# microsoft/ctsTraffic

Measured on AMD Instinct MI355X. Metric: GiB/s verified, 64 KiB buffers device-resident; % MI355X HBM roofline, higher is better.
Workload: dtype u8

## Files before the change

ctstraffic_amd/csrc/cts_kernels.hip:

```cpp
#include <hip/hip_runtime.h>

#include <type_traits>

#include "cts_device_util.hpp"
#include "cts_grids.hpp"
#include "cts_internal.hpp"

namespace cts {

typedef uint32_t u32x4 __attribute__((ext_vector_type(4)));

__device__ __forceinline__ uint32_t pattern_byte_dev(uint32_t pos)
{
    pos &= 0xFFFFu;
    return (pos & 1u) ? (pos >> 9) : ((pos >> 1) & 0xFFu);
}

__device__ __forceinline__ u32x4 expected_chunk(uint32_t q, uint32_t sh)
{
    const uint32_t k = q >> 1;
    const uint32_t base = __umul24(k, 0x10001u) + 0x10000u;
    const uint32_t w0 = base & 0x7FFF7FFFu;
    const uint32_t w1 = (base + 0x20002u) & 0x7FFF7FFFu;
    const uint32_t w2 = (base + 0x40004u) & 0x7FFF7FFFu;
    const uint32_t w3 = (base + 0x60006u) & 0x7FFF7FFFu;
    const uint32_t w4 = (base + 0x80008u) & 0x7FFF7FFFu;
    return u32x4{__builtin_amdgcn_alignbyte(w1, w0, sh), __builtin_amdgcn_alignbyte(w2, w1, sh),
                 __builtin_amdgcn_alignbyte(w3, w2, sh), __builtin_amdgcn_alignbyte(w4, w3, sh)};
}

__device__ __forceinline__ uint32_t nonzero_bytes(uint32_t x)
{
    return (((x & 0x7F7F7F7Fu) + 0x7F7F7F7Fu) | x) & 0x80808080u;
}

__device__ __forceinline__ uint32_t low_bytes_mask(int nb)
{
    return (uint32_t)((1ull << (8 * nb)) - 1ull);
}

__device__ __forceinline__ u32x4 range_mask(uint32_t lo, uint32_t hi)
{
    u32x4 m;
#pragma unroll
    for (int w = 0; w < 4; ++w) {
        int a = (int)lo - 4 * w;
        int b = (int)hi - 4 * w;
        a = a < 0 ? 0 : (a > 4 ? 4 : a);
        b = b < 0 ? 0 : (b > 4 ? 4 : b);
        m[w] = (b > a) ? (low_bytes_mask(b) & ~low_bytes_mask(a)) : 0u;
    }
    return m;
}

template <bool NT>
__device__ __forceinline__ u32x4 load_chunk(const u32x4* p)
{
    if constexpr (NT) {
        return __builtin_nontemporal_load(p);
    } else {
        return *p;
    }
}

__device__ __forceinline__ uint32_t or4(u32x4 x) { return x[0] | x[1] | x[2] | x[3]; }

typedef const u32x4 __attribute__((address_space(1)))* gchunk_ptr;
template <bool NT>
__device__ __forceinline__ u32x4 load_chunk_g(const u32x4* p)
{
    const gchunk_ptr g = (gchunk_ptr)p;
    if constexpr (NT) {
        return __builtin_nontemporal_load(g);
    } else {
        return *g;
    }
}

struct Span {
    const u32x4* p;
    const uint8_t* sp;
    uint32_t len;
    uint32_t nchunks;
    uint32_t q0;
    uint32_t sh;
    uint32_t lo;
    uint32_t hi_last;
    uint32_t expected;
    uint32_t cb0;
};

__device__ __forceinline__ Span make_span(const uint8_t* __restrict__ arena, const cts_buf_desc& d)
{
    Span s;
    s.len = d.length - d.skip_head;
    s.sp = arena + d.byte_offset + d.skip_head;
    s.lo = (uint32_t)((uintptr_t)s.sp & 15u);
    s.nchunks = s.len == 0 ? 0u : (uint32_t)(((uint64_t)s.lo + s.len + 15u) >> 4);
    s.hi_last = s.len == 0 ? 0u : (uint32_t)((uint64_t)s.lo + s.len - 16ull * (s.nchunks - 1u));
    s.q0 = (d.expected_pattern_offset - s.lo) & 0xFFFFu;
    s.sh = s.q0 & 1u;
    s.p = reinterpret_cast<const u32x4*>(s.sp - s.lo);
    s.expected = d.expected_pattern_offset;
    const uint32_t a = (uint32_t)(((uintptr_t)s.p >> 4) & 7u);
    s.cb0 = 8u - a;
    return s;
}

__device__ __forceinline__ u32x4 chunk_xor(const Span& s, uint32_t c, u32x4 data)
{
    return data ^ expected_chunk((s.q0 + 16u * c) & 0xFFFFu, s.sh);
}

__device__ __forceinline__ u32x4 chunk_diff_masked(const Span& s, uint32_t c)
{
    u32x4 x = chunk_xor(s, c, s.p[c]);
    if (c == 0u || c == s.nchunks - 1u) x &= range_mask(c == 0u ? s.lo : 0u, c == s.nchunks - 1u ? s.hi_last : 16u);
    return x;
}

__device__ __forceinline__ __amdgpu_buffer_rsrc_t span_rsrc(const Span& s)
{
    return __builtin_amdgcn_make_buffer_rsrc(const_cast<u32x4*>(s.p), (short)0, (int)(s.nchunks * 16u), 0x00020000);
}

template <bool NT>
__device__ __forceinline__ u32x4 buf_load(__amdgpu_buffer_rsrc_t r, uint32_t voff, uint32_t soff)
{
    return __builtin_amdgcn_raw_buffer_load_b128(r, voff, soff, NT ? 2 : 0);
}

template <int TEAM, int U, bool EVEN = false>
__device__ __forceinline__ u32x4 expected_step(uint32_t B, int u, uint32_t sh)
{
    static_assert(32767 + 8 * TEAM * (U - 1) + 8 < 65536, "packed k must not carry");
    uint32_t bb = B;
    asm volatile("" : "+v"(bb));
    const uint32_t b = bb + (uint32_t)u * (uint32_t)(8 * TEAM) * 0x10001u;
    const uint32_t w0 = b & 0x7FFF7FFFu;
    const uint32_t w1 = (b + 0x20002u) & 0x7FFF7FFFu;
    const uint32_t w2 = (b + 0x40004u) & 0x7FFF7FFFu;
    const uint32_t w3 = (b + 0x60006u) & 0x7FFF7FFFu;
    if constexpr (EVEN) {
        return u32x4{w0, w1, w2, w3};
    } else {
        const uint32_t w4 = (b + 0x80008u) & 0x7FFF7FFFu;
        return u32x4{__builtin_amdgcn_alignbyte(w1, w0, sh), __builtin_amdgcn_alignbyte(w2, w1, sh),
                     __builtin_amdgcn_alignbyte(w3, w2, sh), __builtin_amdgcn_alignbyte(w4, w3, sh)};
    }
}

__device__ __forceinline__ uint32_t chunk_base(const Span& s, uint32_t c)
{
    const uint32_t k = ((s.q0 + 16u * c) & 0xFFFFu) >> 1;
    return __umul24(k, 0x10001u) + 0x10000u;
}

template <int TEAM, int U, bool NT, bool EVEN>
__device__ __forceinline__ uint32_t scan_rounds(const Span& s, __amdgpu_buffer_rsrc_t r, uint32_t lane, uint32_t cb,
                                                uint32_t c_end)
{
    uint32_t acc = 0;
    const uint32_t voff = lane * 16u;
    for (; cb + (uint32_t)(TEAM * U) <= c_end; cb += (uint32_t)(TEAM * U)) {
        u32x4 d[U];
#pragma unroll
        for (int u = 0; u < U; ++u) d[u] = buf_load<NT>(r, voff, (cb + (uint32_t)(u * TEAM)) * 16u);
        __builtin_amdgcn_sched_barrier(0);
        const uint32_t B = chunk_base(s, cb + lane);
#pragma unroll
        for (int u = 0; u < U; ++u) {
            acc |= or4(d[u] ^ expected_step<TEAM, U, EVEN>(B, u, s.sh));
            __builtin_amdgcn_sched_barrier(0);
        }
    }
    if (cb < c_end) {
        u32x4 d[U];
#pragma unroll
        for (int u = 0; u < U; ++u) d[u] = buf_load<NT>(r, (cb + (uint32_t)(u * TEAM) + lane) * 16u, 0u);
        __builtin_amdgcn_sched_barrier(0);
        const uint32_t B = chunk_base(s, cb + lane);
#pragma unroll
        for (int u = 0; u < U; ++u) {
            const uint32_t any = or4(d[u] ^ expected_step<TEAM, U, EVEN>(B, u, s.sh));
            acc |= (cb + (uint32_t)(u * TEAM) + lane < c_end) ? any : 0u;
            __builtin_amdgcn_sched_barrier(0);
        }
    }
    return acc;
}

template <int TEAM, int U, bool NT, bool EVEN>
__device__ __forceinline__ uint32_t scan_interior_impl(const Span& s, __amdgpu_buffer_rsrc_t r, uint32_t lane)
{
    if (s.nchunks < 3u) return 0;
    return scan_rounds<TEAM, U, NT, EVEN>(s, r, lane, s.cb0, s.nchunks - 1u);
}

template <int TEAM, int U, bool NT, bool SPLIT>
__device__ __forceinline__ uint32_t scan_interior(const Span& s, __amdgpu_buffer_rsrc_t r, uint32_t lane)
{
    if constexpr (SPLIT) {
        if (__builtin_amdgcn_readfirstlane(s.sh) == 0u) return scan_interior_impl<TEAM, U, NT, true>(s, r, lane);
    }
    return scan_interior_impl<TEAM, U, NT, false>(s, r, lane);
}

__device__ __forceinline__ bool span_whole_lines(const Span& s)
{
    return s.lo == 0u && s.hi_last == 16u && s.cb0 == 8u;
}

__device__ __forceinline__ uint32_t edge_chunk_of(const Span& s, uint32_t lane)
{
    return lane == 1u ? s.nchunks - 1u : ((lane >= 2u && lane <= 8u) ? lane - 1u : 0u);
}
__device__ __forceinline__ bool edge_chunk_used(const Span& s, uint32_t lane)
{
    if (s.nchunks == 0u) return false;
    if (lane == 0u) return true;
    if (lane == 1u) return s.nchunks > 1u;
    const uint32_t h = s.nchunks - 1u < s.cb0 ? s.nchunks - 1u : s.cb0;
    return lane >= 2u && lane <= 8u && lane - 1u < h;
}

template <int TEAM, int U, bool NT, bool SPLIT = false>
__device__ __forceinline__ uint32_t scan_buffer(const Span& s, uint32_t lane)
{
    const __amdgpu_buffer_rsrc_t r = span_rsrc(s);
    const uint32_t ce = edge_chunk_of(s, lane);
    const u32x4 edge = buf_load<NT>(r, edge_chunk_used(s, lane) ? ce * 16u : 0x7FFFFFF0u, 0u);
    uint32_t acc = scan_interior<TEAM, U, NT, SPLIT>(s, r, lane);
    const u32x4 x = chunk_xor(s, ce, edge) & range_mask(ce == 0u ? s.lo : 0u, ce == s.nchunks - 1u ? s.hi_last : 16u);
    acc |= edge_chunk_used(s, lane) ? or4(x) : 0u;
    return acc;
}

__device__ __forceinline__ void take_diff(const Span& s, uint32_t c, u32x4 x, uint32_t& first, uint32_t& count)
{
#pragma unroll
    for (int w = 0; w < 4; ++w) {
        const uint32_t nz = nonzero_bytes(x[w]);
        if (nz) {
            const uint32_t idx = 4u * (uint32_t)w + ((uint32_t)__builtin_ctz(nz) >> 3);
            const uint32_t pos = 16u * c + idx - s.lo;
            first = pos < first ? pos : first;
            count += (uint32_t)__builtin_popcount(nz);
        }
    }
}

template <int TEAM, int U, bool NT>
__device__ __forceinline__ void scan_exact_owned(const Span& s, uint32_t lane, uint32_t& first, uint32_t& count)
{
    if (s.nchunks == 0) return;
    const __amdgpu_buffer_rsrc_t r = span_rsrc(s);
    if (s.nchunks >= 3u) {
        const uint32_t c_end = s.nchunks - 1u;
        for (uint32_t cb = s.cb0; cb < c_end; cb += (uint32_t)(TEAM * U)) {
            u32x4 d[U];
#pragma unroll
            for (int u = 0; u < U; ++u) d[u] = buf_load<NT>(r, (cb + (uint32_t)(u * TEAM) + lane) * 16u, 0u);
#pragma unroll
            for (int u = 0; u < U; ++u) {
                const uint32_t c = cb + (uint32_t)(u * TEAM) + lane;
                if (c < c_end) take_diff(s, c, chunk_xor(s, c, d[u]), first, count);
            }
        }
    }
    if (edge_chunk_used(s, lane)) {
        const uint32_t c = edge_chunk_of(s, lane);
        const u32x4 x = chunk_xor(s, c, buf_load<NT>(r, c * 16u, 0u)) &
                        range_mask(c == 0u ? s.lo : 0u, c == s.nchunks - 1u ? s.hi_last : 16u);
        take_diff(s, c, x, first, count);
    }
}

template <int TEAM, int U, bool EVEN>
__device__ __forceinline__ void whole_exact_round(const Span& s, u32x4 (&d)[U], uint32_t cb, uint32_t lane,
                                                  uint32_t& first, uint32_t& count)
{
    const uint32_t B = chunk_base(s, cb + lane);
    uint32_t any = 0;
#pragma unroll
    for (int u = 0; u < U; ++u) {
        d[u] ^= expected_step<TEAM, U, EVEN>(B, u, s.sh);
        any |= or4(d[u]);
        __builtin_amdgcn_sched_barrier(0);
    }
    if (any != 0u) {
#pragma unroll
        for (int u = 0; u < U; ++u) take_diff(s, cb + (uint32_t)(u * TEAM) + lane, d[u], first, count);
    }
}

template <int TEAM, int U, bool NT, bool EVEN>
__device__ __forceinline__ void scan_whole_exact_impl(const Span& s, __amdgpu_buffer_rsrc_t r, uint32_t lane,
                                                      uint32_t& first, uint32_t& count)
{
    const uint32_t voff = lane * 16u;
    uint32_t cb = 0;
    const uint32_t c_end = s.nchunks;
    for (; cb + (uint32_t)(TEAM * U) <= c_end; cb += (uint32_t)(TEAM * U)) {
        u32x4 d[U];
#pragma unroll
        for (int u = 0; u < U; ++u) d[u] = buf_load<NT>(r, voff, (cb + (uint32_t)(u * TEAM)) * 16u);
        __builtin_amdgcn_sched_barrier(0);
        whole_exact_round<TEAM, U, EVEN>(s, d, cb, lane, first, count);
    }
    if (cb < c_end) {
        u32x4 d[U];
#pragma unroll
        for (int u = 0; u < U; ++u) d[u] = buf_load<NT>(r, (cb + (uint32_t)(u * TEAM) + lane) * 16u, 0u);
        __builtin_amdgcn_sched_barrier(0);
        const uint32_t B = chunk_base(s, cb + lane);
        uint32_t any = 0;
#pragma unroll
        for (int u = 0; u < U; ++u) {
            const bool in = cb + (uint32_t)(u * TEAM) + lane < c_end;
            d[u] = in ? (d[u] ^ expected_step<TEAM, U, EVEN>(B, u, s.sh)) : u32x4{0u, 0u, 0u, 0u};
            any |= or4(d[u]);
            __builtin_amdgcn_sched_barrier(0);
        }
        if (any != 0u) {
#pragma unroll
            for (int u = 0; u < U; ++u) take_diff(s, cb + (uint32_t)(u * TEAM) + lane, d[u], first, count);
        }
    }
}

template <int TEAM, int U, bool NT, bool SPLIT>
__device__ __forceinline__ void scan_whole_exact(const Span& s, uint32_t lane, uint32_t& first, uint32_t& count)
{
    const __amdgpu_buffer_rsrc_t r = span_rsrc(s);
    if constexpr (SPLIT) {
        if (__builtin_amdgcn_readfirstlane(s.sh) == 0u) {
            scan_whole_exact_impl<TEAM, U, NT, true>(s, r, lane, first, count);
            return;
        }
    }
    scan_whole_exact_impl<TEAM, U, NT, false>(s, r, lane, first, count);
}

constexpr uint32_t kGiantChunks = 1u << 27;

__device__ __forceinline__ bool span_giant(const Span& s)
{
    return __builtin_amdgcn_readfirstlane(s.nchunks >= kGiantChunks ? 1u : 0u) != 0u;
}

template <int TEAM, bool NT, uint32_t G = 2>
__device__ __forceinline__ void scan_giant_exact(const Span& s, uint32_t lane, uint32_t& first, uint32_t& count)
{
    for (uint32_t cb = 0; cb < s.nchunks; cb += G * TEAM) {
        u32x4 d[G];
#pragma unroll
        for (uint32_t g = 0; g < G; ++g) {
            const uint32_t c = cb + g * TEAM + lane;
            d[g] = load_chunk_g<NT>(s.p + (c < s.nchunks ? c : 0u));
        }
#pragma unroll
        for (uint32_t g = 0; g < G; ++g) {
            const uint32_t c = cb + g * TEAM + lane;
            if (c < s.nchunks) {
                u32x4 x = chunk_xor(s, c, d[g]);
                if (c == 0u || c == s.nchunks - 1u)
                    x &= range_mask(c == 0u ? s.lo : 0u, c == s.nchunks - 1u ? s.hi_last : 16u);
                take_diff(s, c, x, first, count);
            }
        }
    }
}

__device__ __forceinline__ uint32_t wave_min(uint32_t v)
{
#pragma unroll
    for (int off = 32; off > 0; off >>= 1) {
        const uint32_t o = (uint32_t)__shfl_xor((int)v, off, 64);
        v = o < v ? o : v;
    }
    return v;
}

__device__ __forceinline__ void write_bad(cts_verify_result* results, uint32_t i)
{
    if (results != nullptr) {
        cts_verify_result r;
        r.first_mismatch = 0;
        r.mismatch_bytes = 0;
        r.expected = 0;
        r.actual = 0;
        r.pass = 0;
        r.flags = CTS_RESULT_FLAG_BAD_DESC;
        results[i] = r;
    }
}

__device__ __forceinline__ void finish_buffer(const Span& s, const cts_buf_desc& d, uint32_t i, uint32_t first,
                                              uint32_t count, cts_verify_result* results, uint64_t* tc,
                                              uint32_t* conn_first_fail, uint32_t n_conns,
                                              cts_verify_result* rslot = nullptr, uint32_t base_index = 0u)
{
    const bool pass = (first == kNone);
    if (rslot != nullptr) {
        cts_verify_result r;
        r.first_mismatch = pass ? s.len : first;
        r.mismatch_bytes = pass ? 0u : count;
        r.expected = pass ? 0 : (uint8_t)pattern_byte_dev(s.expected + first);
        r.actual = pass ? 0 : s.sp[first];
        r.pass = pass ? 1 : 0;
        r.flags = 0;
        *rslot = r;
    } else if (results != nullptr) {
        cts_verify_result r;
        r.first_mismatch = pass ? s.len : first;
        r.mismatch_bytes = pass ? 0u : count;
        r.expected = pass ? 0 : (uint8_t)pattern_byte_dev(s.expected + first);
        r.actual = pass ? 0 : s.sp[first];
        r.pass = pass ? 1 : 0;
        r.flags = 0;
        results[i] = r;
    }
    tc[kBytesChecked] += s.len;
    tc[kBuffersChecked] += 1;
    if (pass) {
        tc[kBytesOk] += s.len;
    } else {
        tc[kBuffersFailed] += 1;
        tc[kMismatchedBytes] += count;
        if (conn_first_fail != nullptr && d.conn_index < n_conns &&
            atomicMin(&conn_first_fail[d.conn_index], base_index + i) == 0xFFFFFFFFu)
            tc[kConnectionsFailed] += 1;
    }
}

template <int TEAMS>
__device__ __forceinline__ void zero_counters(uint64_t (*ctr)[kCounterCount])
{
    if (threadIdx.x < (unsigned)(TEAMS * kCounterCount)) ctr[threadIdx.x / kCounterCount][threadIdx.x % kCounterCount] = 0;
    __syncthreads();
}

template <int TEAMS>
__device__ __forceinline__ void flush_counters(uint64_t* counters, uint64_t (*ctr)[kCounterCount])
{
    __syncthreads();
    if (counters == nullptr) return;
    if (threadIdx.x < (unsigned)kCounterCount) {
        uint64_t sum = 0;
#pragma unroll
        for (int t = 0; t < TEAMS; ++t) sum += ctr[t][threadIdx.x];
        if (sum)
            atomicAdd((unsigned long long*)&counters[(blockIdx.x % CTS_COUNTER_SHARDS) * kCounterSlots + threadIdx.x],
                      (unsigned long long)sum);
    }
}

__device__ __forceinline__ void block_reduce_mismatch_with(uint32_t& first, uint32_t& count, uint32_t* red)
{
    const uint32_t wave = threadIdx.x / 64;
    first = wave_min(first);
    count = wave_sum(count);
    if ((threadIdx.x & 63) == 0) {
        red[wave] = first;
        red[kBlock / 64 + wave] = count;
    }
    __syncthreads();
    if (threadIdx.x == 0) {
#pragma unroll
        for (int w = 1; w < kBlock / 64; ++w) {
            first = red[w] < first ? red[w] : first;
            count += red[kBlock / 64 + w];
        }
    }
    __syncthreads();
}

__device__ __forceinline__ void block_reduce_mismatch(uint32_t& first, uint32_t& count)
{
    __shared__ uint32_t red[2 * (kBlock / 64)];
    block_reduce_mismatch_with(first, count, red);
}

constexpr int kWgLoads = 2;

template <bool NT>
__device__ __forceinline__ void verify_wg_body(const uint8_t* __restrict__ arena, uint64_t arena_bytes,
                                               const cts_buf_desc* __restrict__ descs, uint32_t n,
                                               cts_verify_result* __restrict__ results, uint64_t* __restrict__ counters,
                                               uint32_t* __restrict__ conn_first_fail, uint32_t n_conns,
                                               uint32_t base_index)
{
    __shared__ uint64_t ctr[1][kCounterCount];
    const uint32_t lane = threadIdx.x;
    zero_counters<1>(ctr);
    const uint32_t step = gridDim.x;
    uint32_t i = blockIdx.x;
    cts_buf_desc dn;
    if (i < n) dn = descs[i];
    for (; i < n; i = (uint64_t)i + step < n ? i + step : n) {
        const cts_buf_desc d = dn;
        if ((uint64_t)i + step < n) dn = descs[i + step];
        if (desc_bad(d, arena_bytes)) {
            if (lane == 0) write_bad(results, i);
            continue;
        }
        const Span s = make_span(arena, d);
        uint32_t first = kNone, count = 0;
        bool dirty;
        if (span_giant(s)) {
            scan_giant_exact<kBlock, NT>(s, lane, first, count);
            dirty = __builtin_amdgcn_readfirstlane(__syncthreads_or(first != kNone)) != 0;
            if (dirty) block_reduce_mismatch(first, count);
        } else if (__builtin_amdgcn_readfirstlane(span_whole_lines(s) ? 1u : 0u)) {
            scan_whole_exact<kBlock, kWgLoads, NT, true>(s, lane, first, count);
            dirty = __builtin_amdgcn_readfirstlane(__syncthreads_or(first != kNone)) != 0;
            if (dirty) block_reduce_mismatch(first, count);
        } else {
            const uint32_t acc = scan_buffer<kBlock, kWgLoads, NT, true>(s, lane);
            dirty = __builtin_amdgcn_readfirstlane(__syncthreads_or(acc != 0u)) != 0;
            if (dirty) {
                if (acc != 0u) scan_exact_owned<kBlock, 2, NT>(s, lane, first, count);
                block_reduce_mismatch(first, count);
            }
        }
        if (lane == 0)
            finish_buffer(s, d, i, first, count, results, ctr[0], conn_first_fail, n_conns, nullptr, base_index);
    }
    flush_counters<1>(counters, ctr);
}

template <bool NT>
__global__ void __launch_bounds__(kBlock, 4)
    verify_wg_kernel(const uint8_t* __restrict__ arena, uint64_t arena_bytes, const cts_buf_desc* __restrict__ descs,
                     uint32_t n, cts_verify_result* __restrict__ results, uint64_t* __restrict__ counters,
                     uint32_t* __restrict__ conn_first_fail, uint32_t n_conns)
{
    verify_wg_body<NT>(arena, arena_bytes, descs, n, results, counters, conn_first_fail, n_conns, 0u);
}

template <bool NT>
__global__ void __launch_bounds__(kBlock, 4)
    verify_wg_ordinal(const uint8_t* __restrict__ arena, uint64_t arena_bytes, const cts_buf_desc* __restrict__ descs,
                      uint32_t n, cts_verify_result* __restrict__ results, uint64_t* __restrict__ counters,
                      uint32_t* __restrict__ conn_first_fail, uint32_t n_conns, uint32_t base_index)
{
    verify_wg_body<NT>(arena, arena_bytes, descs, n, results, counters, conn_first_fail, n_conns, base_index);
}

__device__ __forceinline__ void take_diff_at(uint32_t c, uint32_t lo, u32x4 x, uint32_t& first, uint32_t& count)
{
#pragma unroll
    for (int w = 0; w < 4; ++w) {
        const uint32_t nz = nonzero_bytes(x[w]);
        if (nz) {
            const uint32_t pos = 16u * c + 4u * (uint32_t)w + ((uint32_t)__builtin_ctz(nz) >> 3) - lo;
            first = pos < first ? pos : first;
            count += (uint32_t)__builtin_popcount(nz);
        }
    }
}

constexpr int kQuadTeam = 16;

struct QSpan {
    const u32x4* p;
    const uint8_t* sp;
    uint32_t len, nch, hi_last, lo, q0, sh;
    int last;
    int cs;
    int c_hi;
};

__device__ __forceinline__ QSpan quad_span(const uint8_t* sp, uint32_t len, uint32_t expected, const void* dummy)
{
    QSpan q;
    q.sp = len ? sp : reinterpret_cast<const uint8_t*>(dummy);
    q.len = len;
    q.lo = (uint32_t)((uintptr_t)q.sp & 15u);
    q.nch = len == 0u ? 0u : (uint32_t)(((uint64_t)q.lo + len + 15u) >> 4);
    q.hi_last = len == 0u ? 0u : (uint32_t)((uint64_t)q.lo + len - 16ull * (q.nch - 1u));
    q.q0 = (expected - q.lo) & 0xFFFFu;
    q.sh = q.q0 & 1u;
    q.p = reinterpret_cast<const u32x4*>(q.sp - q.lo);
    q.last = q.nch == 0u ? 0 : (int)q.nch - 1;
    q.cs = -(int)(((uintptr_t)q.p >> 4) & 7u);
    q.c_hi = (int)q.nch - 2;
    return q;
}

__device__ __forceinline__ bool quad_edge_used(const QSpan& q, uint32_t lane)
{
    return (lane == 0u && q.nch >= 1u) || (lane == 1u && q.nch >= 2u);
}
__device__ __forceinline__ uint32_t quad_edge_chunk(const QSpan& q, uint32_t lane) { return lane == 1u ? (uint32_t)q.last : 0u; }
__device__ __forceinline__ u32x4 quad_edge_xor(const QSpan& q, uint32_t ce, u32x4 data)
{
    return (data ^ expected_chunk((q.q0 + 16u * ce) & 0xFFFFu, q.sh)) &
           range_mask(ce == 0u ? q.lo : 0u, ce == (uint32_t)q.last ? q.hi_last : 16u);
}

template <int U, bool NT>
__device__ __forceinline__ uint32_t quad_scan_interior(const QSpan& q, uint32_t lane)
{
    constexpr int ROUND = kQuadTeam * U;
    uint32_t acc = 0;
    for (int r = 0; __any(q.cs + r * ROUND <= q.c_hi); ++r) {
        const int cb = q.cs + r * ROUND + (int)lane;
        u32x4 dd[U];
#pragma unroll
        for (int u = 0; u < U; ++u) {
            int c = cb + u * kQuadTeam;
            c = c < 0 ? 0 : (c > q.last ? q.last : c);
            dd[u] = load_chunk_g<NT>(q.p + c);
        }
        __builtin_amdgcn_sched_barrier(0);
        const uint32_t k = ((q.q0 + 16u * (uint32_t)cb) & 0xFFFFu) >> 1;
        const uint32_t B = __umul24(k, 0x10001u) + 0x10000u;
#pragma unroll
        for (int u = 0; u < U; ++u) {
            const int c = cb + u * kQuadTeam;
            const uint32_t any = or4(dd[u] ^ expected_step<kQuadTeam, U>(B, u, q.sh));
            acc |= (c >= 1 && c <= q.c_hi) ? any : 0u;
            __builtin_amdgcn_sched_barrier(0);
        }
    }
    return acc;
}

template <bool NT>
__device__ __forceinline__ void quad_scan_exact(const QSpan& q, uint32_t lane, uint32_t& first, uint32_t& count)
{
    for (int c = q.cs + (int)lane; c <= q.c_hi; c += kQuadTeam) {
        if (c >= 1)
            take_diff_at((uint32_t)c, q.lo,
                         load_chunk_g<NT>(q.p + c) ^ expected_chunk((q.q0 + 16u * (uint32_t)c) & 0xFFFFu, q.sh), first,
                         count);
    }
    if (quad_edge_used(q, lane)) {
        const uint32_t ce = quad_edge_chunk(q, lane);
        take_diff_at(ce, q.lo, quad_edge_xor(q, ce, load_chunk_g<NT>(q.p + ce)), first, count);
    }
}

__device__ __forceinline__ void quad_team_reduce(uint32_t& first, uint32_t& count)
{
#pragma unroll
    for (int off = kQuadTeam / 2; off > 0; off >>= 1) {
        const uint32_t of = (uint32_t)__shfl_xor((int)first, off, kQuadTeam);
        first = of < first ? of : first;
        count += (uint32_t)__shfl_xor((int)count, off, kQuadTeam);
    }
}

struct QCounters {
    uint64_t bytes = 0, ok = 0, mism = 0;
    uint32_t bufs = 0, fail = 0, conns = 0;
    __device__ __forceinline__ void add(uint32_t len, bool pass, uint32_t count)
    {
        bytes += len;
        bufs += 1u;
        if (pass) {
            ok += len;
        } else {
            fail += 1u;
            mism += count;
        }
    }
    template <int TEAMS>
    __device__ __forceinline__ void flush(uint64_t (*ctr)[kCounterCount], uint32_t team, uint32_t lane,
                                          uint64_t* counters) const
    {
        if (lane == 0u) {
            ctr[team][kBytesChecked] = bytes;
            ctr[team][kBytesOk] = ok;
            ctr[team][kBuffersChecked] = bufs;
            ctr[team][kBuffersFailed] = fail;
            ctr[team][kMismatchedBytes] = mism;
            ctr[team][kConnectionsFailed] = conns;
        }
        flush_counters<TEAMS>(counters, ctr);
    }
};

struct QuadOut {
    uint32_t res[4][3];
    uint32_t rec[4][8];
};

__device__ __forceinline__ uint32_t result_dw2(uint32_t expected, uint32_t actual, uint32_t pass, uint32_t flags)
{
    return (expected & 0xFFu) | ((actual & 0xFFu) << 8) | (pass << 16) | (flags << 24);
}

template <typename O>
__device__ __forceinline__ void quad_stage_result(O& o, uint32_t t, uint32_t first_mismatch,
                                                  uint32_t mismatch_bytes, uint32_t dw2)
{
    o.res[t][0] = first_mismatch;
    o.res[t][1] = mismatch_bytes;
    o.res[t][2] = dw2;
}

__device__ __forceinline__ void quad_flush_results(const QuadOut& o, uint32_t i, uint32_t n, cts_verify_result* results)
{
    __builtin_amdgcn_wave_barrier();
    const uint64_t i0 = (uint32_t)__builtin_amdgcn_readfirstlane((int)i);
    const uint32_t l = threadIdx.x & 63u;
    if (results != nullptr && l < 12u) {
        const uint32_t t = l / 3u;
        const uint32_t v = o.res[t][l - 3u * t];
        if (i0 + t < n) reinterpret_cast<uint32_t*>(results)[3ull * i0 + l] = v;
    }
    __builtin_amdgcn_wave_barrier();
}

constexpr int kMsRing = 64;

struct QuadStatusOut {
    uint32_t rec[4][4];
};

template <int K, typename SlotT = QuadOut>
struct QuadRing {
    SlotT slot[K];
    uint32_t i0[K];
};

template <int K, int RECDW = 8, typename SlotT = QuadOut>
__device__ __forceinline__ void quad_ring_flush(const QuadRing<K, SlotT>& g, uint32_t m, uint32_t n,
                                                cts_verify_result* results, void* records)
{
    __builtin_amdgcn_wave_barrier();
    const uint32_t l = threadIdx.x & 63u;
    if (records != nullptr) {
#pragma unroll 1
        for (uint32_t k = 0; k < (K * 4u * RECDW + 63u) / 64u; ++k) {
            const uint32_t e = k * 64u + l, j = e / (4u * RECDW), d = e % (4u * RECDW);
            if (j < m) {
                const uint64_t i0 = g.i0[j];
                if (i0 + d / RECDW < n)
                    __hip_atomic_store(reinterpret_cast<uint32_t*>(records) + (uint64_t)RECDW * i0 + d,
                                       g.slot[j].rec[d / RECDW][d % RECDW], __ATOMIC_RELAXED, __HIP_MEMORY_SCOPE_AGENT);
            }
        }
    }
    if constexpr (!std::is_same<SlotT, QuadStatusOut>::value)
    if (results != nullptr) {
#pragma unroll 1
        for (uint32_t k = 0; k < (K * 12u + 63u) / 64u; ++k) {
            const uint32_t e = k * 64u + l, j = e / 12u, d = e - 12u * j;
            if (j < m) {
                const uint64_t i0 = g.i0[j];
                const uint32_t t = d / 3u;
                if (i0 + t < n) reinterpret_cast<uint32_t*>(results)[3ull * i0 + d] = g.slot[j].res[t][d - 3u * t];
            }
        }
    }
    __builtin_amdgcn_wave_barrier();
}

template <int TEAMS>
struct QuadWalk {
    uint32_t i, end;
    uint64_t cbase;
    uint32_t per, team;
    __device__ __forceinline__ QuadWalk(uint32_t n, uint32_t per_, uint32_t team_) : end(n), per(per_), team(team_)
    {
        cbase = (uint64_t)blockIdx.x * per;
        i = cbase + team < (uint64_t)n ? (uint32_t)(cbase + team) : n;
    }
    __device__ __forceinline__ uint32_t next()
    {
        uint64_t nx = (uint64_t)i + TEAMS;
        if (nx - cbase >= per) {
            cbase += (uint64_t)gridDim.x * per;
            nx = cbase + team;
        }
        return nx < (uint64_t)end ? (uint32_t)nx : end;
    }
};

template <bool STRIDED>
__device__ __forceinline__ cts_buf_desc vs_desc(const VSource& src, uint32_t i)
{
    if constexpr (STRIDED) {
        const uint32_t len = src.lens[i];
        return cts_buf_desc{(uint64_t)i * src.stride, len, len <= src.stride ? src.expected : 65536u, src.conn_index,
                            src.skip_head};
    } else {
        return src.descs[i];
    }
}

constexpr int kQuadLoads = 6;

template <bool NT, bool STRIDED>
__global__ void __launch_bounds__(kBlock)
    verify_quad_kernel(const uint8_t* __restrict__ arena, uint64_t arena_bytes, VSource src, uint32_t n,
                       cts_verify_result* __restrict__ results, uint64_t* __restrict__ counters,
                       uint32_t* __restrict__ conn_first_fail, uint32_t n_conns, uint32_t per, uint32_t base_index)
{
    constexpr int TEAMS = kBlock / kQuadTeam;
    __shared__ uint64_t ctr[TEAMS][kCounterCount];
    __shared__ QuadOut qout[kBlock / 64];
    const uint32_t lane = threadIdx.x & (kQuadTeam - 1);
    const uint32_t team = threadIdx.x / kQuadTeam;
    const void* dummy = STRIDED ? static_cast<const void*>(arena)
                                : reinterpret_cast<const void*>(((uintptr_t)src.descs + 15u) & ~(uintptr_t)15u);
    QCounters qc;
    QuadWalk<TEAMS> w(n, per, team);
    cts_buf_desc dn = vs_desc<STRIDED>(src, w.i < n ? w.i : n - 1u);
    while (__any(w.i < w.end)) {
        const uint32_t i = w.i;
        const cts_buf_desc d = dn;
        const uint32_t inext = w.next();
        dn = vs_desc<STRIDED>(src, inext < n ? inext : n - 1u);
        const bool live = i < w.end;
        const bool ok = live && !desc_bad(d, arena_bytes);
        const QSpan q = quad_span(arena + d.byte_offset + d.skip_head, ok ? d.length - d.skip_head : 0u,
                                  d.expected_pattern_offset, dummy);
        const uint32_t ce = quad_edge_chunk(q, lane);
        const u32x4 edge = load_chunk_g<false>(q.p + ce);
        uint32_t acc = quad_scan_interior<kQuadLoads, NT>(q, lane);
        acc |= quad_edge_used(q, lane) ? or4(quad_edge_xor(q, ce, edge)) : 0u;
        uint32_t first = kNone, count = 0;
        if (__any(acc != 0u)) {
            if (acc != 0u) quad_scan_exact<NT>(q, lane, first, count);
            quad_team_reduce(first, count);
        }
        if (lane == 0u && live) {
            QuadOut& o = qout[team >> 2];
            if (!ok) {
                quad_stage_result(o, team & 3u, 0u, 0u, result_dw2(0u, 0u, 0u, CTS_RESULT_FLAG_BAD_DESC));
            } else {
                const bool pass = first == kNone;
                if (results != nullptr)
                    quad_stage_result(o, team & 3u, pass ? q.len : first, pass ? 0u : count,
                                      pass ? result_dw2(0u, 0u, 1u, 0u)
                                           : result_dw2(pattern_byte_dev(d.expected_pattern_offset + first),
                                                        q.sp[first], 0u, 0u));
                qc.add(q.len, pass, count);
                if (!pass && conn_first_fail != nullptr && d.conn_index < n_conns &&
                    atomicMin(&conn_first_fail[d.conn_index], base_index + i) == 0xFFFFFFFFu)
                    qc.conns += 1u;
            }
        }
        quad_flush_results(qout[team >> 2], i, w.end, results);
        w.i = inext;
    }
// ... 1396 lines not shown
```

Baseline: 6660.

## Cut register pressure in workgroup verify kernel to double occupancy bound

```diff
diff --git a/ctstraffic_amd/csrc/cts_kernels.hip b/ctstraffic_amd/csrc/cts_kernels.hip
--- a/ctstraffic_amd/csrc/cts_kernels.hip
+++ b/ctstraffic_amd/csrc/cts_kernels.hip
@@ -224,15 +224,22 @@
     return lane >= 2u && lane <= 8u && lane - 1u < h;
 }
 
+__device__ __forceinline__ uint32_t opaque_lane(uint32_t lane)
+{
+    asm volatile("" : "+v"(lane));
+    return lane;
+}
+
 template <int TEAM, int U, bool NT, bool SPLIT = false>
 __device__ __forceinline__ uint32_t scan_buffer(const Span& s, uint32_t lane)
 {
     const __amdgpu_buffer_rsrc_t r = span_rsrc(s);
-    const uint32_t ce = edge_chunk_of(s, lane);
-    const u32x4 edge = buf_load<NT>(r, edge_chunk_used(s, lane) ? ce * 16u : 0x7FFFFFF0u, 0u);
+    const uint32_t el = opaque_lane(lane);
+    const uint32_t ce = edge_chunk_of(s, el);
+    const u32x4 edge = buf_load<NT>(r, edge_chunk_used(s, el) ? ce * 16u : 0x7FFFFFF0u, 0u);
     uint32_t acc = scan_interior<TEAM, U, NT, SPLIT>(s, r, lane);
     const u32x4 x = chunk_xor(s, ce, edge) & range_mask(ce == 0u ? s.lo : 0u, ce == s.nchunks - 1u ? s.hi_last : 16u);
-    acc |= edge_chunk_used(s, lane) ? or4(x) : 0u;
+    acc |= edge_chunk_used(s, el) ? or4(x) : 0u;
     return acc;
 }
 
@@ -268,8 +275,9 @@
             }
         }
     }
-    if (edge_chunk_used(s, lane)) {
-        const uint32_t c = edge_chunk_of(s, lane);
+    const uint32_t el = opaque_lane(lane);
+    if (edge_chunk_used(s, el)) {
+        const uint32_t c = edge_chunk_of(s, el);
         const u32x4 x = chunk_xor(s, c, buf_load<NT>(r, c * 16u, 0u)) &
                         range_mask(c == 0u ? s.lo : 0u, c == s.nchunks - 1u ? s.hi_last : 16u);
         take_diff(s, c, x, first, count);
@@ -434,6 +442,23 @@
     }
 }
 
+__device__ __forceinline__ void finish_clean(uint32_t len, uint32_t i, cts_verify_result* results, uint64_t* tc)
+{
+    if (results != nullptr) {
+        cts_verify_result r;
+        r.first_mismatch = len;
+        r.mismatch_bytes = 0u;
+        r.expected = 0;
+        r.actual = 0;
+        r.pass = 1;
+        r.flags = 0;
+        results[i] = r;
+    }
+    tc[kBytesChecked] += len;
+    tc[kBuffersChecked] += 1;
+    tc[kBytesOk] += len;
+}
+
 template <int TEAMS>
 __device__ __forceinline__ void zero_counters(uint64_t (*ctr)[kCounterCount])
 {
@@ -484,68 +509,138 @@
 
 constexpr int kWgLoads = 2;
 
-template <bool NT>
+struct VerifyWgArgs {
+    const uint8_t* arena;
+    uint64_t arena_bytes;
+    const cts_buf_desc* descs;
+    uint32_t n;
+    cts_verify_result* results;
+    uint64_t* counters;
+    uint32_t* conn_first_fail;
+    uint32_t n_conns;
+    uint32_t base_index;
+};
+static_assert(offsetof(VerifyWgArgs, results) == 32 && offsetof(VerifyWgArgs, counters) == 40 &&
+                  offsetof(VerifyWgArgs, conn_first_fail) == 48 && offsetof(VerifyWgArgs, n_conns) == 56 &&
+                  offsetof(VerifyWgArgs, base_index) == 60,
+              "the kernels' argument lists, as the compiler lays them out");
+
+template <typename T>
+__device__ __forceinline__ T kernarg_read(size_t offset)
+{
+    typedef const uint8_t __attribute__((address_space(4)))* kbytes;
+    kbytes p = (kbytes)__builtin_amdgcn_kernarg_segment_ptr();
+    asm volatile("" : "+s"(p));
+    return *(const T __attribute__((address_space(4)))*)(p + offset);
+}
+template <typename T>
+__device__ __forceinline__ T* opaque_global(T* p)
+{
+    uint64_t v = (uint64_t)p;
+    asm volatile("" : "+s"(v));
+    return (T*)(T __attribute__((address_space(1)))*)v;
+}
+#define CTS_WG_ARG(field) kernarg_read<decltype(VerifyWgArgs::field)>(offsetof(VerifyWgArgs, field))
+
+__device__ __forceinline__ uint32_t load_desc_lanes(const cts_buf_desc* __restrict__ descs, uint32_t i, uint32_t lane)
+{
+    static_assert(sizeof(cts_buf_desc) == 24, "six dwords");
+    const uint32_t wl = lane & 63u;
+    const __amdgpu_buffer_rsrc_t r = __builtin_amdgcn_make_buffer_rsrc(const_cast<cts_buf_desc*>(descs + i), (short)0,
+                                                                       (int)sizeof(cts_buf_desc), 0x00020000);
+    return __builtin_amdgcn_raw_buffer_load_b32(r, (wl < 6u ? wl : 5u) * 4u, 0u, 0);
+}
+__device__ __forceinline__ cts_buf_desc desc_from_lanes(uint32_t v)
+{
+    cts_buf_desc d;
+    d.byte_offset = (uint64_t)(uint32_t)__builtin_amdgcn_readlane((int)v, 0) |
+                    (uint64_t)(uint32_t)__builtin_amdgcn_readlane((int)v, 1) << 32;
+    d.length = (uint32_t)__builtin_amdgcn_readlane((int)v, 2);
+    d.expected_pattern_offset = (uint32_t)__builtin_amdgcn_readlane((int)v, 3);
+    d.conn_index = (uint32_t)__builtin_amdgcn_readlane((int)v, 4);
+    d.skip_head = (uint32_t)__builtin_amdgcn_readlane((int)v, 5);
+    return d;
+}
+
+template <bool NT, bool ORDINAL>
 __device__ __forceinline__ void verify_wg_body(const uint8_t* __restrict__ arena, uint64_t arena_bytes,
                                                const cts_buf_desc* __restrict__ descs, uint32_t n,
-                                               cts_verify_result* __restrict__ results, uint64_t* __restrict__ counters,
-                                               uint32_t* __restrict__ conn_first_fail, uint32_t n_conns,
-                                               uint32_t base_index)
+                                               cts_verify_result* __restrict__ results)
 {
     __shared__ uint64_t ctr[1][kCounterCount];
     const uint32_t lane = threadIdx.x;
     zero_counters<1>(ctr);
     const uint32_t step = gridDim.x;
     uint32_t i = blockIdx.x;
-    cts_buf_desc dn;
-    if (i < n) dn = descs[i];
-    for (; i < n; i = (uint64_t)i + step < n ? i + step : n) {
-        const cts_buf_desc d = dn;
-        if ((uint64_t)i + step < n) dn = descs[i + step];
-        if (desc_bad(d, arena_bytes)) {
-            if (lane == 0) write_bad(results, i);
-            continue;
-        }
-        const Span s = make_span(arena, d);
-        uint32_t first = kNone, count = 0;
-        bool dirty;
-        if (span_giant(s)) {
-            scan_giant_exact<kBlock, NT>(s, lane, first, count);
-            dirty = __builtin_amdgcn_readfirstlane(__syncthreads_or(first != kNone)) != 0;
-            if (dirty) block_reduce_mismatch(first, count);
-        } else if (__builtin_amdgcn_readfirstlane(span_whole_lines(s) ? 1u : 0u)) {
-            scan_whole_exact<kBlock, kWgLoads, NT, true>(s, lane, first, count);
-            dirty = __builtin_amdgcn_readfirstlane(__syncthreads_or(first != kNone)) != 0;
-            if (dirty) block_reduce_mismatch(first, count);
+    uint32_t dv = 0;
+    if (i < n) dv = load_desc_lanes(descs, i, lane);
+    cts_buf_desc d = desc_from_lanes(dv);
+    while (i < n) {
+        const bool more = (uint64_t)i + step < n;
+        uint32_t dnv = 0;
+        if (more) dnv = load_desc_lanes(descs, i + step, lane);
+        uint32_t first = kNone, count = 0, len = 0;
+        bool dirty = false;
+        const bool bad = desc_bad(d, arena_bytes);
+        if (!bad) {
+            const Span s = make_span(arena, d);
+            len = s.len;
+            if (span_giant(s)) {
+                scan_giant_exact<kBlock, NT>(s, lane, first, count);
+                dirty = __builtin_amdgcn_readfirstlane(__syncthreads_or(first != kNone)) != 0;
+                if (dirty) block_reduce_mismatch(first, count);
+            } else if (__builtin_amdgcn_readfirstlane(span_whole_lines(s) ? 1u : 0u)) {
+                scan_whole_exact<kBlock, kWgLoads, NT, true>(s, lane, first, count);
+                dirty = __builtin_amdgcn_readfirstlane(__syncthreads_or(first != kNone)) != 0;
+                if (dirty) block_reduce_mismatch(first, count);
+            } else {
+                const uint32_t acc = scan_buffer<kBlock, kWgLoads, NT, true>(s, lane);
+                dirty = __builtin_amdgcn_readfirstlane(__syncthreads_or(acc != 0u)) != 0;
+                if (dirty) {
+                    if (acc != 0u) scan_exact_owned<kBlock, 2, NT>(s, lane, first, count);
+                    block_reduce_mismatch(first, count);
+                }
+            }
+        }
+        uint32_t cur = dv;
+        dv = dnv;
+        d = desc_from_lanes(dv);
+        cts_verify_result* r = opaque_global(results);
+        if (bad) {
+            if (lane == 0) write_bad(r, i);
+        } else if (!dirty) {
+            if (lane == 0) finish_clean(len, i, r, ctr[0]);
         } else {
-            const uint32_t acc = scan_buffer<kBlock, kWgLoads, NT, true>(s, lane);
-            dirty = __builtin_amdgcn_readfirstlane(__syncthreads_or(acc != 0u)) != 0;
-            if (dirty) {
-                if (acc != 0u) scan_exact_owned<kBlock, 2, NT>(s, lane, first, count);
-                block_reduce_mismatch(first, count);
+            asm volatile("" : "+v"(cur));
+            const cts_buf_desc dc = desc_from_lanes(cur);
+            if (lane == 0) {
+                uint32_t base_index = 0u;
+                if constexpr (ORDINAL) base_index = CTS_WG_ARG(base_index);
+                finish_buffer(make_span(arena, dc), dc, i, first, count, r, ctr[0], CTS_WG_ARG(conn_first_fail),
+                              CTS_WG_ARG(n_conns), nullptr, base_index);
             }
         }
-        if (lane == 0)
-            finish_buffer(s, d, i, first, count, results, ctr[0], conn_first_fail, n_conns, nullptr, base_index);
-    }
-    flush_counters<1>(counters, ctr);
+        i = more ? i + step : n;
+    }
+    flush_counters<1>(CTS_WG_ARG(counters), ctr);
 }
 
 template <bool NT>
-__global__ void __launch_bounds__(kBlock, 4)
+__global__ void __launch_bounds__(kBlock, 8)
     verify_wg_kernel(const uint8_t* __restrict__ arena, uint64_t arena_bytes, const cts_buf_desc* __restrict__ descs,
                      uint32_t n, cts_verify_result* __restrict__ results, uint64_t* __restrict__ counters,
                      uint32_t* __restrict__ conn_first_fail, uint32_t n_conns)
 {
-    verify_wg_body<NT>(arena, arena_bytes, descs, n, results, counters, conn_first_fail, n_conns, 0u);
+    verify_wg_body<NT, false>(arena, arena_bytes, descs, n, results);
 }
 
 template <bool NT>
-__global__ void __launch_bounds__(kBlock, 4)
+__global__ void __launch_bounds__(kBlock, 8)
     verify_wg_ordinal(const uint8_t* __restrict__ arena, uint64_t arena_bytes, const cts_buf_desc* __restrict__ descs,
                       uint32_t n, cts_verify_result* __restrict__ results, uint64_t* __restrict__ counters,
                       uint32_t* __restrict__ conn_first_fail, uint32_t n_conns, uint32_t base_index)
 {
-    verify_wg_body<NT>(arena, arena_bytes, descs, n, results, counters, conn_first_fail, n_conns, base_index);
+    verify_wg_body<NT, true>(arena, arena_bytes, descs, n, results);
 }
 
 __device__ __forceinline__ void take_diff_at(uint32_t c, uint32_t lo, u32x4 x, uint32_t& first, uint32_t& count)
```

After: 6646. Within noise of the previous version (-0.2%).
